# Zhen-Dong/HAWQ

Hardware: AMD Instinct MI355X
Metric: images/sec (higher is better)
Workload: dtype int8

## Files before the change

hawq_amd/csrc/fused_wp.hip:

```cpp
#include <stdio.h>
#include <utility>

#include "common.h"

namespace {

struct WPP {
    const uint8_t *x2, *w3, *w1;
    const int32_t *ctab3, *ctab1;
    const uint16_t *res_in;
    uint16_t *res_out;
    uint8_t *y;
    uint8_t *q_out;
    int q_nib;
    int M, C3;
    int m_id_s, e_id_s, mq, eq, q_hi;
    int y_lo, y_hi, y_planar, y_nib;
    int spb;
    int sub, sW, sHW, dW, dHW;
    int32_t *flags;
    long long *dbgbuf;
};

template <int... Is, class Fn>
__device__ __forceinline__ void sfor_impl(std::integer_sequence<int, Is...>, Fn &&f) {
    (f(std::integral_constant<int, Is>{}), ...);
}
template <int N, class Fn>
__device__ __forceinline__ void sfor(Fn &&f) {
    sfor_impl(std::make_integer_sequence<int, N>{}, f);
}

__device__ __forceinline__ void wp_dma16(const char *src, char *dst) {
    __builtin_amdgcn_global_load_lds((const __attribute__((address_space(1))) void *)src, (__attribute__((address_space(3))) void *)dst, 16, 0, 0);
}
__device__ __forceinline__ void wp_dma4(const char *src, char *dst) {
    __builtin_amdgcn_global_load_lds((const __attribute__((address_space(1))) void *)src, (__attribute__((address_space(3))) void *)dst, 4, 0, 0);
}
template <bool K0>
__device__ __forceinline__ DyNt wp_ctab(const char *ctab, int ch) {
    const v4i t = *reinterpret_cast<const v4i *>(ctab + ch * 16);
    DyNt d;
    d.m = t.x, d.s = K0 ? t.y : (t.y & 31), d.k = K0 ? 0 : (t.y >> 8);
    d.add = (long long)(((unsigned long long)(unsigned)t.w << 32) | (unsigned)t.z);
    return d;
}

template <int C_, int NW_, bool REDUCE_, int MINW_>
struct WPCfg {
    static constexpr int C = C_, NW = NW_, MINW = MINW_;
    static constexpr bool REDUCE = REDUCE_;
    static constexpr int NT = 64 * NW, BM = 32 * NW;
    static constexpr int KC = C / 64;
    static constexpr int CT2 = C / 32;
    static constexpr int RPP = NT / 4;
    static constexpr int W3_BYTES = 64 * C;
    static constexpr int W1_BYTES = REDUCE ? 64 * C : 0;
    static constexpr int STAGE = W3_BYTES + W1_BYTES;
    static constexpr int W3PASS = (64 * KC + RPP - 1) / RPP, W1PASS = REDUCE ? (C + RPP - 1) / RPP : 0;
    static constexpr int CTPASS = NW >= 4 ? 1 : 4 / NW;
    static constexpr int NDMA = W3PASS + W1PASS + CTPASS;
    static constexpr int OFF_CT = 2 * STAGE;
    static constexpr int OFF_STG = OFF_CT + 2 * 1024;
    static constexpr int LDS_BYTES = OFF_STG + NW * 4096;
    static_assert(RPP % 16 == 0 && (NW == 1 || NW == 2 || NW % 4 == 0), "producer passes must cover whole swizzle groups");
};

template <class F, bool TIE, bool CK0, bool QK0 = false>
__global__ __launch_bounds__(F::NT, F::MINW) void expand_wp_kernel(const WPP p) {
    extern __shared__ __attribute__((aligned(16))) char smem[];
    constexpr int MODE_S = TIE ? 2 : 0;
    constexpr int MODE_Q = TIE ? 2 : (QK0 ? 1 : 0);
    constexpr int MODE_C = TIE ? 2 : (CK0 ? 1 : 0);
    constexpr bool K0 = CK0 && !TIE;
    constexpr int C = F::C;
    const int t = threadIdx.x, lane = t & 63, wave = t >> 6, l31 = lane & 31, h = lane >> 5;
    const int pix = blockIdx.x * F::BM + wave * 32 + l31;
    const bool valid = pix < p.M;
    const size_t row = valid ? pix : p.M - 1;
    const int nsl = p.C3 >> 6;
    const int j0 = blockIdx.y * p.spb, j1 = (j0 + p.spb < nsl) ? j0 + p.spb : nsl;
    char *ct = smem + F::OFF_CT;
    const int pix0 = blockIdx.x * F::BM + wave * 32;
    auto srow = [&](int d) -> unsigned {
        d = d < p.M ? d : p.M - 1;
        if constexpr (!F::REDUCE) {
            if (p.sub > 1) {
                const int n = d / p.dHW, r = d - n * p.dHW, y = r / p.dW, x = r - y * p.dW;
                return (unsigned)(n * p.sHW + (y * p.sW + x) * p.sub);
            }
        }
        return (unsigned)d;
    };
    unsigned rsrc[4], xsrc[2];
#pragma unroll
    for (int k = 0; k < 4; ++k) rsrc[k] = srow(pix0 + 8 * k + (lane >> 3));
#pragma unroll
    for (int k = 0; k < 2; ++k) xsrc[k] = srow(pix0 + 16 * k + (lane >> 2));
    asm volatile("" : "+v"(rsrc[0]), "+v"(rsrc[1]), "+v"(rsrc[2]), "+v"(rsrc[3]), "+v"(xsrc[0]), "+v"(xsrc[1]));
    const int prow = t >> 2, pslot = t & 3;
    const int sw = (pslot ^ ((prow >> 2) & 3)) << 4;
    auto issue = [&](int j, int stage) {
        char *dst = smem + stage * F::STAGE;
#pragma unroll
        for (int i = 0; i < F::W3PASS; ++i) {
            const int idx = (i * F::RPP + prow) & (64 * F::KC - 1), first = (i * F::RPP + wave * 16) & (64 * F::KC - 1);
            wp_dma16((const char *)p.w3 + (size_t)(j * 64 + (idx & 63)) * C + (idx >> 6) * 64 + sw, dst + first * 64);
        }
#pragma unroll
        for (int i = 0; i < F::W1PASS; ++i) {
            const int r = (i * F::RPP + prow) & (C - 1), first = (i * F::RPP + wave * 16) & (C - 1);
            wp_dma16((const char *)p.w1 + (size_t)r * p.C3 + j * 64 + sw, dst + F::W3_BYTES + first * 64);
        }
#pragma unroll
        for (int i = 0; i < F::CTPASS; ++i) {
            const int q4 = (wave + i * F::NW) & 3;
            wp_dma4((const char *)p.ctab3 + (size_t)j * 1024 + q4 * 256 + lane * 4, ct + (j & 1) * 1024 + q4 * 256);
        }
    };
    char *stg = smem + F::OFF_STG + wave * 4096;
    const int crow = lane >> 3, cslot = lane & 7;
    unsigned coff[4];
#pragma unroll
    for (int k = 0; k < 4; ++k) {
        const int r = 8 * k + crow;
        coff[k] = rsrc[k] * (unsigned)(p.C3 * 2) + ((cslot ^ (r & 7)) << 4);
    }
    auto dma_res = [&](int j) {
#pragma unroll
        for (int k = 0; k < 4; ++k) wp_dma16((const char *)p.res_in + (coff[k] + (unsigned)(j * 128)), stg + k * 1024);
    };
    const unsigned sl = lds_addr(stg) + l31 * 128;
    const int x7 = l31 & 7;
    v4i xf[F::KC][2];
    {
        const int r2 = lane >> 2, s2 = lane & 3;
#pragma unroll
        for (int kc0 = 0; kc0 < F::KC; kc0 += 2) {
#pragma unroll
            for (int kc = kc0; kc < kc0 + 2 && kc < F::KC; ++kc)
#pragma unroll
                for (int k = 0; k < 2; ++k) {
                    const int r = 16 * k + r2;
                    const size_t gr = xsrc[k];
                    wp_dma16((const char *)p.x2 + gr * C + kc * 64 + ((s2 ^ ((r >> 2) & 3)) << 4), stg + (kc - kc0) * 2048 + k * 1024);
                }
            wait_vmcnt<0>();
#pragma unroll
            for (int kc = kc0; kc < kc0 + 2 && kc < F::KC; ++kc)
#pragma unroll
                for (int ks = 0; ks < 2; ++ks)
                    xf[kc][ks] = *reinterpret_cast<const v4i *>(stg + (kc - kc0) * 2048 + lds_off(l31, 2 * ks + h));
            asm volatile("s_waitcnt lgkmcnt(0)" ::: "memory");
#pragma unroll
            for (int kc = kc0; kc < kc0 + 2 && kc < F::KC; ++kc) pin(xf[kc][0]), pin(xf[kc][1]);
        }
    }
    issue(j0, 0);
    dma_res(j0);
    v16i acc2[F::REDUCE ? F::CT2 : 1];
    if constexpr (F::REDUCE) {
#pragma unroll
        for (int c = 0; c < F::CT2; ++c)
#pragma unroll
            for (int r = 0; r < 16; ++r) acc2[c][r] = 0;
    }
    DyNt dids = dynt_prepare(p.m_id_s, p.e_id_s), dq = dynt_prepare(p.mq, p.eq);
    constexpr bool SC0 = QK0 && !TIE;
    DyS0 dis0 = dys0_prepare(p.m_id_s, p.e_id_s);
    asm volatile("" : "+s"(dids.add), "+s"(dq.add), "+s"(dis0.add));
    const unsigned rowmask = valid ? 0xffffffffu : 0u;
    const int qhi2 = (p.q_hi & 0xffff) | (p.q_hi << 16);
    unsigned oor = 0;
    const int cp = cperm(l31);
    const unsigned a0 = lds_addr(smem) + lds_off(cp, h), a1 = lds_addr(smem) + lds_off(cp, 2 + h);
#ifdef HAWQ_ABLATE
    const bool prof = p.dbgbuf != nullptr;
    long long ph[8] = {0, 0, 0, 0, 0, 0, 0, 0};
    long long tprev = prof ? (long long)__builtin_readcyclecounter() : 0;
#define WP_STAMP(K)                                                    \
    if (prof) {                                                        \
        const long long now = (long long)__builtin_readcyclecounter(); \
        ph[K] += now - tprev;                                          \
        tprev = now;                                                   \
    }
#else
#define WP_STAMP(K)
#endif
    for (int j = j0; j < j1; ++j) {
        const int st = (j - j0) & 1;
        wait_vmcnt<4>();
        __builtin_amdgcn_s_barrier();
        WP_STAMP(0)
        const bool more = j + 1 < j1;
        if (more) issue(j + 1, st ^ 1);
        WP_STAMP(1)
        v16i acc1[2];
#pragma unroll
        for (int r = 0; r < 16; ++r) acc1[0][r] = 0, acc1[1][r] = 0;
        {
            const unsigned b0 = a0 + st * F::STAGE, b1 = a1 + st * F::STAGE;
            v4i wf[2][2];
            wf[0][0] = lds_read16<0>(b0), wf[0][1] = lds_read16<2048>(b0);
            sfor<2 * F::KC>([&](auto SI) {
                constexpr int s = decltype(SI)::value, kc = s >> 1, ks = s & 1, cur = s & 1, nxt = cur ^ 1;
                if constexpr (s + 1 < 2 * F::KC) {
                    constexpr int kn = (s + 1) >> 1;
                    wf[nxt][0] = lds_read16<kn * 4096>(ks ? b0 : b1), wf[nxt][1] = lds_read16<kn * 4096 + 2048>(ks ? b0 : b1);
                    wait_lgkm<2>();
                } else {
                    wait_lgkm<0>();
                }
                pin(wf[cur][0]), pin(wf[cur][1]);
                acc1[0] = __builtin_amdgcn_mfma_i32_32x32x32_i8(wf[cur][0], xf[kc][ks], acc1[0], 0, 0, 0);
                acc1[1] = __builtin_amdgcn_mfma_i32_32x32x32_i8(wf[cur][1], xf[kc][ks], acc1[1], 0, 0, 0);
            });
        }
        WP_STAMP(2)
        if (more) wait_vmcnt<F::NDMA>(); else wait_vmcnt<0>();
        v4i rin[4];
        rin[0] = lds_read16<0>(sl + ((4 * 0 + 2 * h) ^ x7) * 16), rin[1] = lds_read16<0>(sl + ((4 * 0 + 2 * h + 1) ^ x7) * 16);
        rin[2] = lds_read16<0>(sl + ((4 * 1 + 2 * h) ^ x7) * 16), rin[3] = lds_read16<0>(sl + ((4 * 1 + 2 * h + 1) ^ x7) * 16);
        wait_lgkm<0>();
        pin(rin[0]), pin(rin[1]), pin(rin[2]), pin(rin[3]);
        WP_STAMP(3)
        v4i qf[2];
        v4i rout[4];
        {
            const char *ctb = ct + (j & 1) * 1024;
#pragma unroll
            for (int tl = 0; tl < 2; ++tl) {
                int qp[4];
#pragma unroll
                for (int g = 0; g < 4; ++g) {
                    const unsigned w0 = (unsigned)rin[2 * tl + (g >> 1)][(g & 1) * 2], w1 = (unsigned)rin[2 * tl + (g >> 1)][(g & 1) * 2 + 1];
                    const int idin[4] = {(int)(w0 & 0xffffu), (int)(w0 >> 16), (int)(w1 & 0xffffu), (int)(w1 >> 16)};
                    int o[4], qv[4];
#pragma unroll
                    for (int k = 0; k < 4; ++k) {
                        const DyNt dm = wp_ctab<K0>(ctb, 32 * tl + 16 * h + 4 * g + k);
                        const int a = dyadic_mode<MODE_C>(acc1[tl][4 * g + k], dm);
                        const int b = SC0 ? dyadic_s0(idin[k], dis0) : dyadic_mode<MODE_S>(idin[k], dids);
                        o[k] = max(a + b, 0);
                        qv[k] = dyadic_mode<MODE_Q>(o[k], dq);
                    }
                    oor |= ((unsigned)(o[0] | o[1]) | (unsigned)(o[2] | o[3])) & rowmask;
                    rout[2 * tl + (g >> 1)][(g & 1) * 2] = pack2_u16_sat(o[0], o[1]);
                    rout[2 * tl + (g >> 1)][(g & 1) * 2 + 1] = pack2_u16_sat(o[2], o[3]);
                    qp[g] = pack4_min(qv[0], qv[1], qv[2], qv[3], qhi2);
                }
                qf[tl] = v4i{qp[0], qp[1], qp[2], qp[3]};
            }
        }
        WP_STAMP(4)
        if (p.res_out) {
            *reinterpret_cast<v4i *>(stg + l31 * 128 + ((4 * 0 + 2 * h) ^ x7) * 16) = rout[0];
            *reinterpret_cast<v4i *>(stg + l31 * 128 + ((4 * 0 + 2 * h + 1) ^ x7) * 16) = rout[1];
            *reinterpret_cast<v4i *>(stg + l31 * 128 + ((4 * 1 + 2 * h) ^ x7) * 16) = rout[2];
            *reinterpret_cast<v4i *>(stg + l31 * 128 + ((4 * 1 + 2 * h + 1) ^ x7) * 16) = rout[3];
#pragma unroll
            for (int k = 0; k < 4; ++k) {
                const int r = 8 * k + crow;
                const v4i v = *reinterpret_cast<const v4i *>(stg + k * 1024 + lane * 16);
                if (pix0 + r < p.M) *reinterpret_cast<v4i *>((char *)p.res_out + (coff[k] + (unsigned)(j * 128))) = v;
            }
        }
        if constexpr (!F::REDUCE) {
            if (p.q_out && p.q_nib) {
                asm volatile("s_waitcnt lgkmcnt(0)" ::: "memory");
#pragma unroll
                for (int tl = 0; tl < 2; ++tl)
                    *reinterpret_cast<v2i *>(stg + l31 * 32 + 16 * tl + 8 * h) = v2i{qf[tl].x | (qf[tl].y << 4), qf[tl].z | (qf[tl].w << 4)};
                const int r = lane >> 1, s2 = lane & 1;
                const v4i v = *reinterpret_cast<const v4i *>(stg + lane * 16);
                if (pix0 + r < p.M)
                    *reinterpret_cast<v4i *>((char *)p.q_out + (size_t)(pix0 + r) * (p.C3 >> 1) + j * 32 + s2 * 16) = v;
            } else if (p.q_out) {
                asm volatile("s_waitcnt lgkmcnt(0)" ::: "memory");
                *reinterpret_cast<v4i *>(stg + lds_off(l31, h)) = qf[0];
                *reinterpret_cast<v4i *>(stg + lds_off(l31, 2 + h)) = qf[1];
                const int r2 = lane >> 2, s2 = lane & 3;
#pragma unroll
                for (int k = 0; k < 2; ++k) {
                    const int r = 16 * k + r2;
                    const v4i v = *reinterpret_cast<const v4i *>(stg + k * 1024 + lane * 16);
                    if (pix0 + r < p.M)
                        *reinterpret_cast<v4i *>((char *)p.q_out + (size_t)(pix0 + r) * p.C3 + j * 64 + ((s2 ^ ((r >> 2) & 3)) << 4)) = v;
                }
            }
        }
        asm volatile("s_waitcnt lgkmcnt(0)" ::: "memory");
        if (more) dma_res(j + 1);
        WP_STAMP(5)
        if constexpr (F::REDUCE) {
            const unsigned b0 = a0 + st * F::STAGE + F::W3_BYTES, b1 = a1 + st * F::STAGE + F::W3_BYTES;
            v4i wf[2][2];
            wf[0][0] = lds_read16<0>(b0), wf[0][1] = lds_read16<0>(b1);
            sfor<F::CT2>([&](auto CI) {
                constexpr int c = decltype(CI)::value, cur = c & 1, nxt = cur ^ 1;
                if constexpr (c + 1 < F::CT2) {
                    wf[nxt][0] = lds_read16<(c + 1) * 2048>(b0), wf[nxt][1] = lds_read16<(c + 1) * 2048>(b1);
                    wait_lgkm<2>();
                } else {
                    wait_lgkm<0>();
                }
                pin(wf[cur][0]), pin(wf[cur][1]);
                acc2[c] = __builtin_amdgcn_mfma_i32_32x32x32_i8(wf[cur][0], qf[0], acc2[c], 0, 0, 0);
                acc2[c] = __builtin_amdgcn_mfma_i32_32x32x32_i8(wf[cur][1], qf[1], acc2[c], 0, 0, 0);
            });
        }
        WP_STAMP(6)
    }
#ifdef HAWQ_ABLATE
    if (prof && blockIdx.x == 8 && blockIdx.y == 0 && t == 0)
        for (int k = 0; k < 8; ++k) p.dbgbuf[k] = ph[k];
#endif
#undef WP_STAMP
    if ((oor >> 16) != 0) atomicOr(p.flags, 1);
    if constexpr (F::REDUCE) {
        wait_vmcnt<0>();
#pragma unroll
        for (int c = 0; c < F::CT2; ++c) {
            const int ch0 = 32 * c + 16 * h;
            int w[4];
#pragma unroll
            for (int g = 0; g < 4; ++g) {
                int qv[4];
#pragma unroll
                for (int k = 0; k < 4; ++k)
                    qv[k] = med3i(dyadic_mode<MODE_C>(acc2[c][4 * g + k], wp_ctab<K0>((const char *)p.ctab1, ch0 + 4 * g + k)), p.y_lo, p.y_hi);
                w[g] = pack4_fast(qv[0], qv[1], qv[2], qv[3]);
            }
            const v4i ww = {w[0], w[1], w[2], w[3]};
            if (valid && p.y_nib) {
                const v2i nn = {w[0] | (w[1] << 4), w[2] | (w[3] << 4)};
                if (p.y_planar)
                    *reinterpret_cast<v2i *>((char *)p.y + ((size_t)(ch0 >> 5) * p.M + row) * 16 + ((ch0 >> 4) & 1) * 8) = nn;
                else
                    *reinterpret_cast<v2i *>((char *)p.y + row * (C / 2) + (ch0 >> 1)) = nn;
            } else if (valid) {
                if (p.y_planar)
                    *reinterpret_cast<v4i *>((char *)p.y + ((size_t)(ch0 >> 4) * p.M + row) * 16) = ww;
                else
                    *reinterpret_cast<v4i *>((char *)p.y + row * C + ch0) = ww;
            }
        }
    }
}

typedef void (*WPFn)(const WPP);
struct WPInfo { WPFn fn[5]; int c, bm, nt, lds; bool reduce; int ysplit; };
#define WP_ENTRY(F, YS) {{expand_wp_kernel<F, false, false>, expand_wp_kernel<F, false, true>, expand_wp_kernel<F, true, false>, expand_wp_kernel<F, false, true, true>, \
                          expand_wp_kernel<F, false, false, true>}, F::C, F::BM, F::NT, F::LDS_BYTES, F::REDUCE, YS}
using W64 = WPCfg<64, 4, true, 3>;
using W64B = WPCfg<64, 8, true, 3>;
using W128 = WPCfg<128, 4, true, 2>;
using W128B = WPCfg<128, 8, true, 2>;
using W256 = WPCfg<256, 4, true, 1>;
using N64 = WPCfg<64, 4, false, 4>;
using N128 = WPCfg<128, 4, false, 3>;
using N256 = WPCfg<256, 4, false, 3>;
using N512 = WPCfg<512, 4, false, 2>;
const WPInfo kWP[] = {WP_ENTRY(W64, 1), WP_ENTRY(W64B, 1), WP_ENTRY(W128, 1), WP_ENTRY(W128B, 1), WP_ENTRY(W256, 1),
                      WP_ENTRY(N64, 1), WP_ENTRY(N128, 1), WP_ENTRY(N256, 1), WP_ENTRY(N256, 2), WP_ENTRY(N256, 4),
                      WP_ENTRY(N512, 1), WP_ENTRY(N512, 2), WP_ENTRY(N512, 4), WP_ENTRY(N512, 8)};
constexpr int NUM_WP = sizeof(kWP) / sizeof(kWP[0]);

bool wp_expand_ok(const hawq_conv_args &e) {
    return (e.in_pitch == 0 || e.in_pitch == e.Cin) && (e.out_pitch == 0 || e.out_pitch == e.Cout) && e.KH == 1 && e.KW == 1 && e.stride == 1 && e.pad == 0 && e.in_bits == 8 && e.w_bits == 8 && e.fast_tables != 0 && !e.in2 &&
           !e.in_planar && e.epilogue == HAWQ_EPI_RESIDUAL && e.res_in && e.res_in_bits == 16 && (!e.res_out || e.res_out_bits == 16) &&
           e.flags && e.ctab && e.Cout % 64 == 0 && (e.out_bits == 8 || (e.out_bits == 4 && e.q_lo >= 0 && e.q_hi <= 15)) &&
           (e.out_sub < 2 || !e.res_out);
}

int wp_variant(const hawq_expand_reduce_args *a, int nth) {
    const hawq_conv_args &e = a->expand, &r = a->reduce;
    if (!wp_expand_ok(e)) return -1;
    const bool reduce = r.wgt != nullptr;
    if (reduce && e.out_bits != 8) return -1;
    if (reduce && (e.out_sub >= 2 || r.out_sub >= 2)) return -1;
    if (reduce) {
        if (!(r.KH == 1 && r.KW == 1 && r.stride == 1 && r.pad == 0 && r.in_bits == 8 && r.w_bits == 8 && r.fast_tables != 0 && !r.in2)) return -1;
        if (r.epilogue != HAWQ_EPI_REQUANT || !r.ctab || !r.out_q || (r.out_bits != 8 && r.out_bits != 4) || !e.res_out) return -1;
        if (r.out_bits == 4 && (r.q_lo < 0 || r.q_hi > 15)) return -1;
        if (r.Cin != e.Cout || r.Cout != e.Cin || r.N != e.N || r.H != e.H || r.W != e.W) return -1;
    }
    int n = 0;
    for (int i = 0; i < NUM_WP; ++i)
        if (kWP[i].c == e.Cin && kWP[i].reduce == reduce && (e.Cout / 64) % kWP[i].ysplit == 0 && ++n == nth) return i;
    return -1;
}

}

int wp_num_variants(const hawq_expand_reduce_args *a) {
    int n = 0;
    while (wp_variant(a, n + 1) >= 0) ++n;
    return n;
}

int wp_launch(const hawq_expand_reduce_args *a, int nth, void *stream) {
    const int v = wp_variant(a, nth);
    HAWQ_REQUIRE(v >= 0, "hawq_conv_expand_reduce: no wave-private variant %d for this launch", nth);
    const hawq_conv_args &e = a->expand, &r = a->reduce;
    auto e_fast = [](int ek) { return (ek & 0xff) >= 33 && (ek & 0xff) <= 62 && (ek >> 8) >= 0 && (ek >> 8) < 31; };
    HAWQ_REQUIRE(e.mq >= 0 && e_fast(e.eq) && e.m_id_scalar >= 0 && e_fast(e.e_id_scalar), "hawq_conv_expand_reduce: scalar tables outside the fast contract");
    HAWQ_REQUIRE(e.q_lo <= 0, "hawq_conv_expand_reduce: the block-input QuantAct clamp must admit 0");
    const WPInfo &wi = kWP[v];
    WPP p;
    p.x2 = (const uint8_t *)e.in, p.w3 = (const uint8_t *)e.wgt, p.w1 = (const uint8_t *)r.wgt;
    p.ctab3 = e.ctab, p.ctab1 = wi.reduce ? r.ctab : nullptr;
    p.res_in = (const uint16_t *)e.res_in, p.res_out = (uint16_t *)e.res_out;
    p.y = wi.reduce ? (uint8_t *)r.out_q : nullptr;
    p.q_out = wi.reduce ? nullptr : (uint8_t *)e.out_q;
    p.q_nib = !wi.reduce && e.out_bits == 4;
    const int sub = e.out_sub >= 2 ? e.out_sub : 1, hd = (e.H - 1) / sub + 1, wd = (e.W - 1) / sub + 1;
    const long long Msrc = (long long)e.N * e.H * e.W, M = (long long)e.N * hd * wd;
    HAWQ_REQUIRE(M > 0 && Msrc * e.Cout * 2 < (1ll << 32), "hawq_conv_expand_reduce: bad problem size");
    p.M = (int)M, p.C3 = e.Cout;
    p.sub = sub, p.sW = e.W, p.sHW = e.H * e.W, p.dW = wd, p.dHW = hd * wd;
    p.m_id_s = e.m_id_scalar, p.e_id_s = e.e_id_scalar, p.mq = e.mq, p.eq = e.eq, p.q_hi = e.q_hi;
    p.y_lo = wi.reduce ? (r.relu && r.q_lo < 0 ? 0 : r.q_lo) : 0, p.y_hi = wi.reduce ? r.q_hi : 0;
    p.y_planar = wi.reduce ? r.out_planar : 0;
    p.y_nib = wi.reduce && r.out_bits == 4;
    p.spb = (e.Cout / 64) / wi.ysplit;
    p.flags = e.flags;
    p.dbgbuf = nullptr;
#ifdef HAWQ_ABLATE
    static const int dbg_env = HAWQ_DBG_ENV();
    static long long *dbg_dev = nullptr;
    if ((dbg_env & 128) && !dbg_dev) (void)hipMalloc(&dbg_dev, 8 * sizeof(long long));
    if (dbg_env & 128) p.dbgbuf = dbg_dev;
#endif
    static const bool attrs = [] {
        bool good = true;
        for (const WPInfo &k : kWP)
            for (int i = 0; i < 5; ++i)
                good &= hipFuncSetAttribute((const void *)k.fn[i], hipFuncAttributeMaxDynamicSharedMemorySize, k.lds) == hipSuccess;
        return good;
    }();
    HAWQ_REQUIRE(attrs, "hawq_conv_expand_reduce: hipFuncSetAttribute(MaxDynamicSharedMemorySize) failed");
    const int ft = e.fast_tables | (wi.reduce ? r.fast_tables : 0);
    const bool tie = (ft & 4) != 0, ck0 = (e.fast_tables & 8) && (!wi.reduce || (r.fast_tables & 8));
    const bool qk0 = (e.eq >> 8) == 0 && ids0_form(e.e_id_scalar);
    HAWQ_REQUIRE(e.q_hi >= 0 && e.q_hi <= 32767, "hawq_conv_expand_reduce: q_hi outside [0, 32767]");
    hipLaunchKernelGGL(wi.fn[tie ? 2 : (ck0 ? (qk0 ? 3 : 1) : (qk0 ? 4 : 0))], dim3((p.M + wi.bm - 1) / wi.bm, wi.ysplit), dim3(wi.nt), wi.lds, (hipStream_t)stream, p);
    HAWQ_CHECK_HIP(hipGetLastError());
    if (p.dbgbuf) {
        long long hb[8];
        (void)hipStreamSynchronize((hipStream_t)stream);
        (void)hipMemcpy(hb, p.dbgbuf, sizeof(hb), hipMemcpyDeviceToHost);
        fprintf(stderr, "[wave-private C=%d bm=%d reduce=%d ysplit=%d M=%d C3=%d] cycles of wave 0 / workgroup 8 over %d slices: wait+barrier %lld | issue ring DMA %lld | "
                        "GEMM1 %lld | wait + read residual %lld | epilogue %lld | stage + store + residual DMA %lld | GEMM2 %lld\n",
                wi.c, wi.bm, (int)wi.reduce, wi.ysplit, p.M, p.C3, p.spb, hb[0], hb[1], hb[2], hb[3], hb[4], hb[5], hb[6]);
    }
    return 0;
}
```

hawq_amd/engine.py:

```python
from __future__ import annotations

import ctypes as C
import os
import sys
from functools import partial

import numpy as np
import torch

from . import _lib, packing
from . import plan as _plan
from .plan import ChainChoice, StalePlan
from .quant_utils import requant_table, tables_are_fast, tables_fit_fast
from .runner import EventTimer, GraphRunner, _act_range, _i32, two_round_min


RES_VBITS = 20
U16_VBITS = 17


def out_sub_stride(readers) -> int:
    readers = list(readers)
    if not readers:
        return 0
# ... 337 lines not shown
            return True
        if in_bits != c.w_bits or c.band() is None:
            return False
        q.wgt_band, q.in_planar, q.ctab = c.band().data_ptr(), 1, 1
        if is_last:
            q.res_out_bits, q.flags, q.res_out = 16, 1, 1
        return _lib.load().hawq_conv2d_band2_tile(C.byref(q)) != 0

    def _try_fuse(self, a, u, nxt, N, ho, wo, keep):
        if nxt is None or nxt['resize'] or len(nxt['convs']) != 3 or not a.fast_tables:
            return None
        if int(u['name'].split('.')[0][len('stage'):]) not in self.fuse_stages:
            return None
        ent = nxt['convs'][0]
        c = ent['conv']
        if not ent.get('fast', False) or ent['out_bits'] not in (4, 8) or a.in_bits != 8 or a.w_bits != 8:
            return None
        ob = ent['out_bits']
        er = _lib.ExpandReduceArgs()
        C.memmove(C.byref(er.expand), C.byref(a), C.sizeof(a))
        er.expand.out_q, er.expand.out_bits = None, 8
        r = er.reduce
        if c.w_bits != 8 and not hasattr(c, "w8"):
            c.w8 = torch.from_numpy(packing.pack_conv_weight(c.w_host, 8)).to(self.dev)
        r.wgt, r.bias = (c.w if c.w_bits == 8 else c.w8).data_ptr(), c.bias.data_ptr()
        if c.w_bits == 8 and c.k128() is not None:
            r.wgt_k128 = c.k128().data_ptr()
        r.N, r.H, r.W, r.Cin, r.Cout, r.KH, r.KW, r.stride, r.pad = N, ho, wo, c.cin, c.cout, c.kh, c.kw, c.stride, c.pad
        r.in_bits, r.w_bits = 8, 8
        r.m, r.e, r.ctab = ent['m'].data_ptr(), ent['e'].data_ptr(), ent['ctab'].data_ptr()
        r.flags = self.flags.data_ptr()
        r.epilogue, r.relu = _lib.EPI_REQUANT, 1
        r.out_bits, r.q_lo, r.q_hi = ob, ent['rng'][0], ent['rng'][1]
        r.fast_tables = (5 if ent.get('tie', False) else 1) | (8 if ent.get('ck0', False) else 0)
        r.out_q = 1
        if _lib.load().hawq_conv_expand_reduce_variants(C.byref(er)) == 0:
            return None
        out = self._alloc(N * ho * wo * c.cout * ob // 8, torch.uint8)
        r.out_q = out.data_ptr()
        planar = self.planar and self._band_takes(nxt['convs'][1], N, ho, wo, ob, False, nxt)
        r.out_planar = int(planar)
        q = self._alloc(N * ho * wo * c.cin * nxt['a_bits'] // 8, torch.uint8)
        a.out_q = q.data_ptr()
        r1 = _lib.ConvArgs()
        C.memmove(C.byref(r1), C.byref(r), C.sizeof(r1))
        r1.in_, r1.in_bits = q.data_ptr(), nxt['a_bits']
        r1.wgt, r1.w_bits = c.w.data_ptr(), c.w_bits
        r1.wgt_k128 = c.k128().data_ptr() if (c.k128() is not None and c.w_bits == nxt['a_bits']) else None
        pair = _FusedPair(er, a, r1, self.stream.cuda_stream, self._ws)
        keep += [out, er, q, r1, pair]
        return pair, out, ob, planar

    def _try_solo(self, a, u, keep):
        if not a.fast_tables or a.in2 or os.environ.get("HAWQ_NO_SOLO"):
            return None
        er = _lib.ExpandReduceArgs()
        C.memmove(C.byref(er.expand), C.byref(a), C.sizeof(a))
        if _lib.load().hawq_conv_expand_reduce_variants(C.byref(er)) == 0:
            return None
        pair = _FusedPair(er, a, None, self.stream.cuda_stream, self._ws)
        keep += [er, pair]
        return pair

    def _alloc(self, n, dtype):
        return torch.empty(n, dtype=dtype, device=self.dev)

    def _build(self, N, H, W):
        self._build_plan(N, H, W)
        if not os.environ.get("HAWQ_KEEP_PACKED"):
            self._release_unused_weights()

    def _release_unused_weights(self):
        lib = _lib.load()
        n, nb2, ng2 = lib.hawq_conv2d_num_tiles(), lib.hawq_conv2d_num_band2_tiles(), lib.hawq_conv2d_num_gemm2_tiles()
        band_ids, gemm_ids = range(n - ng2 - nb2 + 1, n - ng2 + 1), range(n - ng2 + 1, n + 1)
        args = []
        for e in (self.subs or [self]):
            args += list(e._conv_args)
            for pr in e._er_args:
                if not pr.fused:
                    args += [pr.expand] + ([pr.reduce] if pr.reduce is not None else [])
        live_band = {a.wgt_band for a in args if a.wgt_band and (a.tile in band_ids or a.tile == 0)}
        live_k128 = {ptr for a in args if (a.tile in gemm_ids or a.tile == 0) for ptr in (a.wgt_k128, a.wgt2_k128) if ptr}
        every = []
        for e in (self.subs or [self]):
            every += list(e._conv_args)
            for pr in e._er_args:
                every += [pr.expand, pr.er.expand, pr.er.reduce] + ([pr.reduce] if pr.reduce is not None else [])
        for a in every:
            if a.wgt_band and a.wgt_band not in live_band:
                a.wgt_band = None
            if a.wgt_k128 and a.wgt_k128 not in live_k128:
                a.wgt_k128 = None
            if a.wgt2_k128 and a.wgt2_k128 not in live_k128:
                a.wgt2_k128 = None
        convs = [c for u in self.P['units'] for c in [ent['conv'] for ent in u['convs']] + ([u['ident']] if u['resize'] else [])]
        self.packed_weight_bytes = 0
        for c in convs:
            wb, wk = c._w_band, c._w_k128
            c.release(wb is not None and wb.data_ptr() not in live_band, wk is not None and wk.data_ptr() not in live_k128)
            self.packed_weight_bytes += sum(t.numel() for t in (c._w_band, c._w_k128) if t is not None)

    def _build_plan(self, N, H, W):
        self._plan_on = bool(self.plan) and int(self.plan.get("batch", -1)) == N and not self.keep_acc
        self.chains = max(1, self.chains_req)
        if self._plan_on:
            try:
# ... 258 lines not shown
                    planar_next = bool(a.fast_tables) and self.planar and self._band_takes(u['convs'][ci + 1], N, ho, wo, xb_next,
                                                                                            ci + 1 == len(u['convs']) - 1, u)
                    a.out_planar = int(planar_next)
                else:
                    a.epilogue = _lib.EPI_RESIDUAL
                    if u['resize']:
                        ic = u['ident']
                        a.in2, a.wgt2, a.bias2 = qa.data_ptr(), ic.w.data_ptr(), ic.bias.data_ptr()
                        if u['a_bits'] == ic.w_bits and ic.k128() is not None:
                            a.wgt2_k128 = ic.k128().data_ptr()
                        a.H2, a.W2, a.Cin2, a.stride2 = h, w, ic.cin, (1 if sub_in else ic.stride)
                        a.in2_bits, a.w2_bits = u['a_bits'], ic.w_bits
                        a.m_id, a.e_id = u['m_id'].data_ptr(), u['e_id'].data_ptr()
                    else:
                        a.res_in, a.res_in_bits = res.data_ptr(), res_bits_in
                        a.m_id_scalar, a.e_id_scalar = u['m_id_s'], u['e_id_s']
                    need_res = (nxt is None) or (not nxt['resize'])
                    new_res = self._alloc(N * ho * wo * c.cout, rdt) if need_res else None
                    if sub_out:
                        a.out_sub = sub_out
                        qh, qw = out_sub_extent(ho, sub_out), out_sub_extent(wo, sub_out)
                    else:
                        qh, qw = ho, wo
                    if new_res is not None:
                        a.res_out, a.res_out_bits = new_res.data_ptr(), self.res_bits
                        self.res_taps[u['name']] = (new_res, (N, ho, wo, c.cout))
                    new_qa = None
                    if nxt is not None:
                        a.out_bits = nxt['a_bits']
                        a.q_lo, a.q_hi, a.mq, a.eq = nxt['a_rng'][0], nxt['a_rng'][1], nxt['mq'], nxt['eq']
                    keep.append(new_res)
                if self.keep_acc:
                    self._add_acc_tap(ops, keep, a, tap_name, N, ho, wo, c.cout)
                    if ci == len(u['convs']) - 1 and u['resize']:
                        self._add_ident_tap(ops, keep, u, qa, N, h, w, ho, wo)
                keep.append(a)
                fz = self._try_fuse(a, u, nxt, N, ho, wo, keep) if (ci == len(u['convs']) - 1 and not self.keep_acc) else None
                if fz is None and ci == len(u['convs']) - 1 and nxt is not None:
                    new_qa = self._alloc(N * qh * qw * c.cout * nxt['a_bits'] // 8, torch.uint8)
                    a.out_q = new_qa.data_ptr()
                    keep.append(new_qa)
                if fz is not None:
                    pair, fout, fbits, fplanar = fz
                    fused_in = (fout, fbits, fplanar)
                    self._er_args.append(pair)
                    self._er_names.append(tap_name)
                    ops.next_name = tap_name + "+" + nxt['name'] + ".quant_convbn1"
                    ops.append(pair)
                    continue
                solo = self._try_solo(a, u, keep) if (ci == len(u['convs']) - 1 and not self.keep_acc) else None
                if solo is not None:
                    self._er_args.append(solo)
                    self._er_names.append(tap_name + "@solo")
                    ops.next_name = tap_name
                    ops.append(solo)
                    continue
                self._conv_args.append(a)
                self._conv_names.append(tap_name)
                self._conv_ops.append(_ConvLaunch(a, self._ws, sp))
                ops.next_name = tap_name + ("+identity" if (a.in2 is not None) else "")
                ops.append(self._conv_ops[-1])
                if ci < len(u['convs']) - 1:
                    x_in, x_bits, hin, win, x_planar = x_next, xb_next, ho, wo, planar_next
            res, qa, h, w = new_res, new_qa, qh, qw
            res_bits_in = self.res_bits
        cl = units[-1]['convs'][-1]['conv'].cout
        qf = self._alloc(N * cl, torch.int8)
        pooled = self._alloc(N * cl, torch.int32) if self.keep_acc else None
        if pooled is not None:
            self.acc_taps['final_pool'] = (pooled, (N, cl))
        o = P['out']
        ops.append(partial(_lib.call, "hawq_avgpool_requant", res.data_ptr(), self.res_bits, N, h * w, cl, qf.data_ptr(),
                           ptr(pooled), o['mq'], o['eq'], o['rng'][0], o['rng'][1], sp))
        fc = P['fc']
        if fc['k'] != cl:
            raise RuntimeError("FC input width does not match the last stage")
        self.logits = logits_view if logits_view is not None else torch.empty(N, fc['nout'], dtype=torch.float32, device=dev)
        a = _lib.ConvArgs()
        a.in_, a.wgt, a.bias = qf.data_ptr(), fc['w'].data_ptr(), fc['bias'].data_ptr()
        a.N, a.H, a.W, a.Cin, a.Cout, a.KH, a.KW, a.stride, a.pad = N, 1, 1, fc['k'], fc['nout_p'], 1, 1, 1, 0
        a.in_bits, a.w_bits = 8, 8
        a.epilogue = _lib.EPI_DEQUANT
        a.out_f32, a.fscale, a.ldo, a.n_valid = self.logits.data_ptr(), fc['fscale'].data_ptr(), fc['nout'], fc['nout']
        if self.keep_acc:
            self._add_acc_tap(ops, keep, a, 'quant_output', N, 1, 1, fc['nout_p'])
        ops.next_name = "quant_output"
        if _lib.load().hawq_fc_dequant_ok(N, fc['k'], fc['nout_p']) and not os.environ.get("HAWQ_NO_FC2"):
            ops.append(partial(_lib.call, "hawq_fc_dequant", qf.data_ptr(), fc['w'].data_ptr(), fc['bias'].data_ptr(), fc['fscale'].data_ptr(),
                               self.logits.data_ptr(), N, fc['k'], fc['nout_p'], fc['nout'], fc['nout'], sp))
        else:
            self._conv_ops.append(_ConvLaunch(a, self._ws, sp))
            ops.append(self._conv_ops[-1])
            self._conv_args.append(a)
            self._conv_names.append("quant_output")
        keep += [qf, pooled, a]
        self._ops, self._keep, self._batch = ops, keep, (N, H, W)
        self._graph = None
        if self.autotune and not self.keep_acc:
            ch = _plan.decode(fixed, chain, self._conv_names, len(self._er_args), int(_lib.load().hawq_conv2d_num_tiles()), self._variant_counts())
            self._apply_choice(self._time_choice(ch) if ch.tiles is None else ch)

    def _add_acc_tap(self, ops, keep, a, name, N, ho, wo, cout):
        acc = self._alloc(N * ho * wo * cout, torch.int32)
        r = _lib.ConvArgs()
        C.memmove(C.byref(r), C.byref(a), C.sizeof(r))
        r.in2 = None
        r.epilogue, r.out_acc = _lib.EPI_RAW, acc.data_ptr()
# ... 246 lines not shown
```

Measured before the change: 104,200.

## Fuse downsample identity conv into wave-private expand kernel via dual GEMM

Adds a DUAL variant of the wave-private expand kernel that computes the downsample/identity 1x1 conv (second input and weights, optionally strided) alongside the main expand GEMM. The two MFMA streams are interleaved in one loop, and each has its own requant table. This lets blocks whose last conv carries an identity branch (in2) take the solo fused path instead of the generic conv kernel. It also switches output stores to nontemporal in that variant, at the cost of more LDS, more registers and a full vmcnt wait per slice.

```diff
diff --git a/hawq_amd/csrc/fused_wp.hip b/hawq_amd/csrc/fused_wp.hip
--- a/hawq_amd/csrc/fused_wp.hip
+++ b/hawq_amd/csrc/fused_wp.hip
@@ -1,4 +1,5 @@
 #include <stdio.h>
+#include <stdlib.h>
 #include <utility>
 
 #include "common.h"
@@ -7,7 +8,8 @@
 
 struct WPP {
     const uint8_t *x2, *w3, *w1;
-    const int32_t *ctab3, *ctab1;
+    const uint8_t *xid, *wid;
+    const int32_t *ctab3, *ctab1, *ctab_id;
     const uint16_t *res_in;
     uint16_t *res_out;
     uint8_t *y;
@@ -18,6 +20,7 @@
     int y_lo, y_hi, y_planar, y_nib;
     int spb;
     int sub, sW, sHW, dW, dHW;
+    int s2, sW2, sHW2;
     int32_t *flags;
     long long *dbgbuf;
 };
@@ -36,6 +39,10 @@
 }
 __device__ __forceinline__ void wp_dma4(const char *src, char *dst) {
     __builtin_amdgcn_global_load_lds((const __attribute__((address_space(1))) void *)src, (__attribute__((address_space(3))) void *)dst, 4, 0, 0);
+}
+template <bool NT>
+__device__ __forceinline__ void wp_store(v4i *dst, const v4i &v) {
+    if constexpr (NT) __builtin_nontemporal_store(v, dst); else *dst = v;
 }
 template <bool K0>
 __device__ __forceinline__ DyNt wp_ctab(const char *ctab, int ch) {
@@ -46,25 +53,38 @@
     return d;
 }
 
-template <int C_, int NW_, bool REDUCE_, int MINW_>
+template <int C_, int NW_, bool REDUCE_, int MINW_, int K2_ = 0>
 struct WPCfg {
-    static constexpr int C = C_, NW = NW_, MINW = MINW_;
-    static constexpr bool REDUCE = REDUCE_;
+    static constexpr int C = C_, NW = NW_, MINW = MINW_, K2 = K2_;
+    static constexpr bool REDUCE = REDUCE_, DUAL = K2_ > 0;
     static constexpr int NT = 64 * NW, BM = 32 * NW;
     static constexpr int KC = C / 64;
     static constexpr int CT2 = C / 32;
     static constexpr int RPP = NT / 4;
     static constexpr int W3_BYTES = 64 * C;
     static constexpr int W1_BYTES = REDUCE ? 64 * C : 0;
-    static constexpr int STAGE = W3_BYTES + W1_BYTES;
+    static constexpr int KC2 = K2 / 64;
+    static constexpr int WID_BYTES = 64 * K2;
+    static constexpr int OFF_WID = W3_BYTES + W1_BYTES;
+    static constexpr int STAGE = W3_BYTES + W1_BYTES + WID_BYTES;
     static constexpr int W3PASS = (64 * KC + RPP - 1) / RPP, W1PASS = REDUCE ? (C + RPP - 1) / RPP : 0;
+    static constexpr int WIDPASS = (64 * KC2 + RPP - 1) / RPP;
     static constexpr int CTPASS = NW >= 4 ? 1 : 4 / NW;
-    static constexpr int NDMA = W3PASS + W1PASS + CTPASS;
+    static constexpr int NDMA = W3PASS + W1PASS + WIDPASS + (DUAL ? 2 : 1) * CTPASS;
     static constexpr int OFF_CT = 2 * STAGE;
-    static constexpr int OFF_STG = OFF_CT + 2 * 1024;
+    static constexpr int OFF_STG = OFF_CT + (DUAL ? 4 : 2) * 1024;
     static constexpr int LDS_BYTES = OFF_STG + NW * 4096;
     static_assert(RPP % 16 == 0 && (NW == 1 || NW == 2 || NW % 4 == 0), "producer passes must cover whole swizzle groups");
+    static_assert(K2 % 64 == 0 && (!DUAL || 64 * KC2 >= RPP), "an identity pass may not be wider than the identity slice");
 };
+
+constexpr int wp_merge(int i, int S1, int S2) {
+    int a = 0, b = 0;
+    for (int n = 0; n < i; ++n) {
+        if (b >= S2 || (a < S1 && a * S2 <= b * S1)) ++a; else ++b;
+    }
+    return (b >= S2 || (a < S1 && a * S2 <= b * S1)) ? a : 256 + b;
+}
 
 template <class F, bool TIE, bool CK0, bool QK0 = false>
 __global__ __launch_bounds__(F::NT, F::MINW) void expand_wp_kernel(const WPP p) {
@@ -117,6 +137,18 @@
             const int q4 = (wave + i * F::NW) & 3;
             wp_dma4((const char *)p.ctab3 + (size_t)j * 1024 + q4 * 256 + lane * 4, ct + (j & 1) * 1024 + q4 * 256);
         }
+        if constexpr (F::DUAL) {
+#pragma unroll
+            for (int i = 0; i < F::WIDPASS; ++i) {
+                const int idx = (i * F::RPP + prow) & (64 * F::KC2 - 1), first = (i * F::RPP + wave * 16) & (64 * F::KC2 - 1);
+                wp_dma16((const char *)p.wid + (size_t)(j * 64 + (idx & 63)) * F::K2 + (idx >> 6) * 64 + sw, dst + F::OFF_WID + first * 64);
+            }
+#pragma unroll
+            for (int i = 0; i < F::CTPASS; ++i) {
+                const int q4 = (wave + i * F::NW) & 3;
+                wp_dma4((const char *)p.ctab_id + (size_t)j * 1024 + q4 * 256 + lane * 4, ct + 2048 + (j & 1) * 1024 + q4 * 256);
+            }
+        }
     };
     char *stg = smem + F::OFF_STG + wave * 4096;
     const int crow = lane >> 3, cslot = lane & 7;
@@ -156,8 +188,43 @@
             for (int kc = kc0; kc < kc0 + 2 && kc < F::KC; ++kc) pin(xf[kc][0]), pin(xf[kc][1]);
         }
     }
+    v4i xid[F::DUAL ? F::KC2 : 1][2];
+    if constexpr (F::DUAL) {
+        const int r2 = lane >> 2, s2 = lane & 3;
+        unsigned xsrc2[2];
+#pragma unroll
+        for (int k = 0; k < 2; ++k) {
+            int d = pix0 + 16 * k + r2;
+            d = d < p.M ? d : p.M - 1;
+            if (p.s2 > 1) {
+                const int n = d / p.dHW, r = d - n * p.dHW, y = r / p.dW, x = r - y * p.dW;
+                d = n * p.sHW2 + (y * p.sW2 + x) * p.s2;
+            }
+            xsrc2[k] = (unsigned)d;
+        }
+#pragma unroll
+        for (int kc0 = 0; kc0 < F::KC2; kc0 += 2) {
+#pragma unroll
+            for (int kc = kc0; kc < kc0 + 2 && kc < F::KC2; ++kc)
+#pragma unroll
+                for (int k = 0; k < 2; ++k) {
+                    const int r = 16 * k + r2;
+                    const size_t gr = xsrc2[k];
+                    wp_dma16((const char *)p.xid + gr * F::K2 + kc * 64 + ((s2 ^ ((r >> 2) & 3)) << 4), stg + (kc - kc0) * 2048 + k * 1024);
+                }
+            wait_vmcnt<0>();
+#pragma unroll
+            for (int kc = kc0; kc < kc0 + 2 && kc < F::KC2; ++kc)
+#pragma unroll
+                for (int ks = 0; ks < 2; ++ks)
+                    xid[kc][ks] = *reinterpret_cast<const v4i *>(stg + (kc - kc0) * 2048 + lds_off(l31, 2 * ks + h));
+            asm volatile("s_waitcnt lgkmcnt(0)" ::: "memory");
+#pragma unroll
+            for (int kc = kc0; kc < kc0 + 2 && kc < F::KC2; ++kc) pin(xid[kc][0]), pin(xid[kc][1]);
+        }
+    }
     issue(j0, 0);
-    dma_res(j0);
+    if constexpr (!F::DUAL) dma_res(j0);
     v16i acc2[F::REDUCE ? F::CT2 : 1];
     if constexpr (F::REDUCE) {
 #pragma unroll
@@ -165,10 +232,15 @@
 #pragma unroll
             for (int r = 0; r < 16; ++r) acc2[c][r] = 0;
     }
-    DyNt dids = dynt_prepare(p.m_id_s, p.e_id_s), dq = dynt_prepare(p.mq, p.eq);
+    DyNt dids{}, dq = dynt_prepare(p.mq, p.eq);
     constexpr bool SC0 = QK0 && !TIE;
-    DyS0 dis0 = dys0_prepare(p.m_id_s, p.e_id_s);
-    asm volatile("" : "+s"(dids.add), "+s"(dq.add), "+s"(dis0.add));
+    DyS0 dis0{};
+    if constexpr (!F::DUAL) {
+        dids = dynt_prepare(p.m_id_s, p.e_id_s), dis0 = dys0_prepare(p.m_id_s, p.e_id_s);
+        asm volatile("" : "+s"(dids.add), "+s"(dq.add), "+s"(dis0.add));
+    } else {
+        asm volatile("" : "+s"(dq.add));
+    }
     const unsigned rowmask = valid ? 0xffffffffu : 0u;
     const int qhi2 = (p.q_hi & 0xffff) | (p.q_hi << 16);
     unsigned oor = 0;
@@ -189,16 +261,44 @@
 #endif
     for (int j = j0; j < j1; ++j) {
         const int st = (j - j0) & 1;
-        wait_vmcnt<4>();
+        if constexpr (F::DUAL) wait_vmcnt<0>(); else wait_vmcnt<4>();
         __builtin_amdgcn_s_barrier();
         WP_STAMP(0)
         const bool more = j + 1 < j1;
         if (more) issue(j + 1, st ^ 1);
         WP_STAMP(1)
-        v16i acc1[2];
+        v16i acc1[2], accid[F::DUAL ? 2 : 1];
 #pragma unroll
         for (int r = 0; r < 16; ++r) acc1[0][r] = 0, acc1[1][r] = 0;
-        {
+        if constexpr (F::DUAL) {
+#pragma unroll
+            for (int r = 0; r < 16; ++r) accid[0][r] = 0, accid[1][r] = 0;
+            const unsigned b0 = a0 + st * F::STAGE, b1 = a1 + st * F::STAGE;
+            constexpr int S1 = 2 * F::KC, S2 = 2 * F::KC2;
+            auto frag = [&](auto EI, v4i &f0, v4i &f1) {
+                constexpr int e = decltype(EI)::value, g = e >> 8, s = e & 255, off = (g ? F::OFF_WID : 0) + (s >> 1) * 4096;
+                f0 = lds_read16<off>((s & 1) ? b1 : b0), f1 = lds_read16<off + 2048>((s & 1) ? b1 : b0);
+            };
+            v4i wf[2][2];
+            frag(std::integral_constant<int, wp_merge(0, S1, S2)>{}, wf[0][0], wf[0][1]);
+            sfor<S1 + S2>([&](auto SI) {
+                constexpr int i = decltype(SI)::value, e = wp_merge(i, S1, S2), g = e >> 8, s = e & 255, cur = i & 1, nxt = cur ^ 1;
+                if constexpr (i + 1 < S1 + S2) {
+                    frag(std::integral_constant<int, wp_merge(i + 1, S1, S2)>{}, wf[nxt][0], wf[nxt][1]);
+                    wait_lgkm<2>();
+                } else {
+                    wait_lgkm<0>();
+                }
+                pin(wf[cur][0]), pin(wf[cur][1]);
+                if constexpr (g == 0) {
+                    acc1[0] = __builtin_amdgcn_mfma_i32_32x32x32_i8(wf[cur][0], xf[s >> 1][s & 1], acc1[0], 0, 0, 0);
+                    acc1[1] = __builtin_amdgcn_mfma_i32_32x32x32_i8(wf[cur][1], xf[s >> 1][s & 1], acc1[1], 0, 0, 0);
+                } else {
+                    accid[0] = __builtin_amdgcn_mfma_i32_32x32x32_i8(wf[cur][0], xid[s >> 1][s & 1], accid[0], 0, 0, 0);
+                    accid[1] = __builtin_amdgcn_mfma_i32_32x32x32_i8(wf[cur][1], xid[s >> 1][s & 1], accid[1], 0, 0, 0);
+                }
+            });
+        } else {
             const unsigned b0 = a0 + st * F::STAGE, b1 = a1 + st * F::STAGE;
             v4i wf[2][2];
             wf[0][0] = lds_read16<0>(b0), wf[0][1] = lds_read16<2048>(b0);
@@ -217,12 +317,14 @@
             });
         }
         WP_STAMP(2)
-        if (more) wait_vmcnt<F::NDMA>(); else wait_vmcnt<0>();
-        v4i rin[4];
-        rin[0] = lds_read16<0>(sl + ((4 * 0 + 2 * h) ^ x7) * 16), rin[1] = lds_read16<0>(sl + ((4 * 0 + 2 * h + 1) ^ x7) * 16);
-        rin[2] = lds_read16<0>(sl + ((4 * 1 + 2 * h) ^ x7) * 16), rin[3] = lds_read16<0>(sl + ((4 * 1 + 2 * h + 1) ^ x7) * 16);
-        wait_lgkm<0>();
-        pin(rin[0]), pin(rin[1]), pin(rin[2]), pin(rin[3]);
+        v4i rin[F::DUAL ? 1 : 4];
+        if constexpr (!F::DUAL) {
+            if (more) wait_vmcnt<F::NDMA>(); else wait_vmcnt<0>();
+            rin[0] = lds_read16<0>(sl + ((4 * 0 + 2 * h) ^ x7) * 16), rin[1] = lds_read16<0>(sl + ((4 * 0 + 2 * h + 1) ^ x7) * 16);
+            rin[2] = lds_read16<0>(sl + ((4 * 1 + 2 * h) ^ x7) * 16), rin[3] = lds_read16<0>(sl + ((4 * 1 + 2 * h + 1) ^ x7) * 16);
+            wait_lgkm<0>();
+            pin(rin[0]), pin(rin[1]), pin(rin[2]), pin(rin[3]);
+        }
         WP_STAMP(3)
         v4i qf[2];
         v4i rout[4];
@@ -233,14 +335,22 @@
                 int qp[4];
 #pragma unroll
                 for (int g = 0; g < 4; ++g) {
-                    const unsigned w0 = (unsigned)rin[2 * tl + (g >> 1)][(g & 1) * 2], w1 = (unsigned)rin[2 * tl + (g >> 1)][(g & 1) * 2 + 1];
-                    const int idin[4] = {(int)(w0 & 0xffffu), (int)(w0 >> 16), (int)(w1 & 0xffffu), (int)(w1 >> 16)};
+                    int idin[4];
+                    if constexpr (!F::DUAL) {
+                        const unsigned w0 = (unsigned)rin[2 * tl + (g >> 1)][(g & 1) * 2], w1 = (unsigned)rin[2 * tl + (g >> 1)][(g & 1) * 2 + 1];
+                        idin[0] = (int)(w0 & 0xffffu), idin[1] = (int)(w0 >> 16), idin[2] = (int)(w1 & 0xffffu), idin[3] = (int)(w1 >> 16);
+                    }
                     int o[4], qv[4];
+                    if constexpr (F::DUAL) __builtin_amdgcn_sched_barrier(0);
 #pragma unroll
                     for (int k = 0; k < 4; ++k) {
                         const DyNt dm = wp_ctab<K0>(ctb, 32 * tl + 16 * h + 4 * g + k);
                         const int a = dyadic_mode<MODE_C>(acc1[tl][4 * g + k], dm);
-                        const int b = SC0 ? dyadic_s0(idin[k], dis0) : dyadic_mode<MODE_S>(idin[k], dids);
+                        int b;
+                        if constexpr (F::DUAL)
+                            b = dyadic_mode<MODE_C>(accid[tl][4 * g + k], wp_ctab<K0>(ctb + 2048, 32 * tl + 16 * h + 4 * g + k));
+                        else
+                            b = SC0 ? dyadic_s0(idin[k], dis0) : dyadic_mode<MODE_S>(idin[k], dids);
                         o[k] = max(a + b, 0);
                         qv[k] = dyadic_mode<MODE_Q>(o[k], dq);
                     }
@@ -262,7 +372,7 @@
             for (int k = 0; k < 4; ++k) {
                 const int r = 8 * k + crow;
                 const v4i v = *reinterpret_cast<const v4i *>(stg + k * 1024 + lane * 16);
-                if (pix0 + r < p.M) *reinterpret_cast<v4i *>((char *)p.res_out + (coff[k] + (unsigned)(j * 128))) = v;
+                if (pix0 + r < p.M) wp_store<F::DUAL>(reinterpret_cast<v4i *>((char *)p.res_out + (coff[k] + (unsigned)(j * 128))), v);
             }
         }
         if constexpr (!F::REDUCE) {
@@ -285,12 +395,14 @@
                     const int r = 16 * k + r2;
                     const v4i v = *reinterpret_cast<const v4i *>(stg + k * 1024 + lane * 16);
                     if (pix0 + r < p.M)
-                        *reinterpret_cast<v4i *>((char *)p.q_out + (size_t)(pix0 + r) * p.C3 + j * 64 + ((s2 ^ ((r >> 2) & 3)) << 4)) = v;
+                        wp_store<F::DUAL>(reinterpret_cast<v4i *>((char *)p.q_out + (size_t)(pix0 + r) * p.C3 + j * 64 + ((s2 ^ ((r >> 2) & 3)) << 4)), v);
                 }
             }
         }
         asm volatile("s_waitcnt lgkmcnt(0)" ::: "memory");
-        if (more) dma_res(j + 1);
+        if constexpr (!F::DUAL) {
+            if (more) dma_res(j + 1);
+        }
         WP_STAMP(5)
         if constexpr (F::REDUCE) {
             const unsigned b0 = a0 + st * F::STAGE + F::W3_BYTES, b1 = a1 + st * F::STAGE + F::W3_BYTES;
@@ -349,9 +461,11 @@
 }
 
 typedef void (*WPFn)(const WPP);
-struct WPInfo { WPFn fn[5]; int c, bm, nt, lds; bool reduce; int ysplit; };
+struct WPInfo { WPFn fn[5]; int c, k2, bm, nt, lds; bool reduce; int ysplit; };
 #define WP_ENTRY(F, YS) {{expand_wp_kernel<F, false, false>, expand_wp_kernel<F, false, true>, expand_wp_kernel<F, true, false>, expand_wp_kernel<F, false, true, true>, \
-                          expand_wp_kernel<F, false, false, true>}, F::C, F::BM, F::NT, F::LDS_BYTES, F::REDUCE, YS}
+                          expand_wp_kernel<F, false, false, true>}, F::C, 0, F::BM, F::NT, F::LDS_BYTES, F::REDUCE, YS}
+#define WP_DUAL_ENTRY(F, YS) {{expand_wp_kernel<F, false, false>, expand_wp_kernel<F, false, true>, expand_wp_kernel<F, true, false>, nullptr, nullptr}, \
+                              F::C, F::K2, F::BM, F::NT, F::LDS_BYTES, F::REDUCE, YS}
 using W64 = WPCfg<64, 4, true, 3>;
 using W64B = WPCfg<64, 8, true, 3>;
 using W128 = WPCfg<128, 4, true, 2>;
@@ -361,14 +475,23 @@
 using N128 = WPCfg<128, 4, false, 3>;
 using N256 = WPCfg<256, 4, false, 3>;
 using N512 = WPCfg<512, 4, false, 2>;
+using D128 = WPCfg<128, 4, false, 2, 256>;
 const WPInfo kWP[] = {WP_ENTRY(W64, 1), WP_ENTRY(W64B, 1), WP_ENTRY(W128, 1), WP_ENTRY(W128B, 1), WP_ENTRY(W256, 1),
                       WP_ENTRY(N64, 1), WP_ENTRY(N128, 1), WP_ENTRY(N256, 1), WP_ENTRY(N256, 2), WP_ENTRY(N256, 4),
-                      WP_ENTRY(N512, 1), WP_ENTRY(N512, 2), WP_ENTRY(N512, 4), WP_ENTRY(N512, 8)};
+                      WP_ENTRY(N512, 1), WP_ENTRY(N512, 2), WP_ENTRY(N512, 4), WP_ENTRY(N512, 8),
+                      WP_DUAL_ENTRY(D128, 1), WP_DUAL_ENTRY(D128, 2)};
 constexpr int NUM_WP = sizeof(kWP) / sizeof(kWP[0]);
 
+bool wp_dual_ok(const hawq_conv_args &e) {
+    const char *off = getenv("HAWQ_NO_WP_DUAL");
+    return !(off && *off) && e.wgt2 && e.ctab_id && e.in2_bits == 8 && e.w2_bits == 8 && e.stride2 >= 1 && e.H2 >= 1 && e.W2 >= 1 &&
+           (e.H2 - 1) / e.stride2 + 1 == e.H && (e.W2 - 1) / e.stride2 + 1 == e.W &&
+           !e.res_in && e.out_sub < 2 && e.out_bits == 8;
+}
+
 bool wp_expand_ok(const hawq_conv_args &e) {
-    return (e.in_pitch == 0 || e.in_pitch == e.Cin) && (e.out_pitch == 0 || e.out_pitch == e.Cout) && e.KH == 1 && e.KW == 1 && e.stride == 1 && e.pad == 0 && e.in_bits == 8 && e.w_bits == 8 && e.fast_tables != 0 && !e.in2 &&
-           !e.in_planar && e.epilogue == HAWQ_EPI_RESIDUAL && e.res_in && e.res_in_bits == 16 && (!e.res_out || e.res_out_bits == 16) &&
+    return (e.in_pitch == 0 || e.in_pitch == e.Cin) && (e.out_pitch == 0 || e.out_pitch == e.Cout) && e.KH == 1 && e.KW == 1 && e.stride == 1 && e.pad == 0 && e.in_bits == 8 && e.w_bits == 8 && e.fast_tables != 0 &&
+           !e.in_planar && e.epilogue == HAWQ_EPI_RESIDUAL && (e.in2 ? wp_dual_ok(e) : (e.res_in && e.res_in_bits == 16)) && (!e.res_out || e.res_out_bits == 16) &&
            e.flags && e.ctab && e.Cout % 64 == 0 && (e.out_bits == 8 || (e.out_bits == 4 && e.q_lo >= 0 && e.q_hi <= 15)) &&
            (e.out_sub < 2 || !e.res_out);
 }
@@ -385,9 +508,11 @@
         if (r.out_bits == 4 && (r.q_lo < 0 || r.q_hi > 15)) return -1;
         if (r.Cin != e.Cout || r.Cout != e.Cin || r.N != e.N || r.H != e.H || r.W != e.W) return -1;
     }
+    const int k2 = e.in2 ? e.Cin2 : 0;
+    if (e.in2 && k2 <= 0) return -1;
     int n = 0;
     for (int i = 0; i < NUM_WP; ++i)
-        if (kWP[i].c == e.Cin && kWP[i].reduce == reduce && (e.Cout / 64) % kWP[i].ysplit == 0 && ++n == nth) return i;
+        if (kWP[i].c == e.Cin && kWP[i].k2 == k2 && kWP[i].reduce == reduce && (e.Cout / 64) % kWP[i].ysplit == 0 && ++n == nth) return i;
     return -1;
 }
 
@@ -404,11 +529,13 @@
     HAWQ_REQUIRE(v >= 0, "hawq_conv_expand_reduce: no wave-private variant %d for this launch", nth);
     const hawq_conv_args &e = a->expand, &r = a->reduce;
     auto e_fast = [](int ek) { return (ek & 0xff) >= 33 && (ek & 0xff) <= 62 && (ek >> 8) >= 0 && (ek >> 8) < 31; };
-    HAWQ_REQUIRE(e.mq >= 0 && e_fast(e.eq) && e.m_id_scalar >= 0 && e_fast(e.e_id_scalar), "hawq_conv_expand_reduce: scalar tables outside the fast contract");
+    const bool dual = e.in2 != nullptr;
+    HAWQ_REQUIRE(e.mq >= 0 && e_fast(e.eq) && (dual || (e.m_id_scalar >= 0 && e_fast(e.e_id_scalar))), "hawq_conv_expand_reduce: scalar tables outside the fast contract");
     HAWQ_REQUIRE(e.q_lo <= 0, "hawq_conv_expand_reduce: the block-input QuantAct clamp must admit 0");
     const WPInfo &wi = kWP[v];
     WPP p;
     p.x2 = (const uint8_t *)e.in, p.w3 = (const uint8_t *)e.wgt, p.w1 = (const uint8_t *)r.wgt;
+    p.xid = (const uint8_t *)e.in2, p.wid = (const uint8_t *)e.wgt2, p.ctab_id = dual ? e.ctab_id : nullptr;
     p.ctab3 = e.ctab, p.ctab1 = wi.reduce ? r.ctab : nullptr;
     p.res_in = (const uint16_t *)e.res_in, p.res_out = (uint16_t *)e.res_out;
     p.y = wi.reduce ? (uint8_t *)r.out_q : nullptr;
@@ -419,6 +546,8 @@
     HAWQ_REQUIRE(M > 0 && Msrc * e.Cout * 2 < (1ll << 32), "hawq_conv_expand_reduce: bad problem size");
     p.M = (int)M, p.C3 = e.Cout;
     p.sub = sub, p.sW = e.W, p.sHW = e.H * e.W, p.dW = wd, p.dHW = hd * wd;
+    p.s2 = dual ? e.stride2 : 1, p.sW2 = e.W2, p.sHW2 = e.H2 * e.W2;
+    HAWQ_REQUIRE(!dual || (long long)e.N * e.H2 * e.W2 * e.Cin2 < (1ll << 32), "hawq_conv_expand_reduce: bad problem size");
     p.m_id_s = e.m_id_scalar, p.e_id_s = e.e_id_scalar, p.mq = e.mq, p.eq = e.eq, p.q_hi = e.q_hi;
     p.y_lo = wi.reduce ? (r.relu && r.q_lo < 0 ? 0 : r.q_lo) : 0, p.y_hi = wi.reduce ? r.q_hi : 0;
     p.y_planar = wi.reduce ? r.out_planar : 0;
@@ -436,13 +565,13 @@
         bool good = true;
         for (const WPInfo &k : kWP)
             for (int i = 0; i < 5; ++i)
-                good &= hipFuncSetAttribute((const void *)k.fn[i], hipFuncAttributeMaxDynamicSharedMemorySize, k.lds) == hipSuccess;
+                good &= !k.fn[i] || hipFuncSetAttribute((const void *)k.fn[i], hipFuncAttributeMaxDynamicSharedMemorySize, k.lds) == hipSuccess;
         return good;
     }();
     HAWQ_REQUIRE(attrs, "hawq_conv_expand_reduce: hipFuncSetAttribute(MaxDynamicSharedMemorySize) failed");
     const int ft = e.fast_tables | (wi.reduce ? r.fast_tables : 0);
     const bool tie = (ft & 4) != 0, ck0 = (e.fast_tables & 8) && (!wi.reduce || (r.fast_tables & 8));
-    const bool qk0 = (e.eq >> 8) == 0 && ids0_form(e.e_id_scalar);
+    const bool qk0 = !dual && (e.eq >> 8) == 0 && ids0_form(e.e_id_scalar);
     HAWQ_REQUIRE(e.q_hi >= 0 && e.q_hi <= 32767, "hawq_conv_expand_reduce: q_hi outside [0, 32767]");
     hipLaunchKernelGGL(wi.fn[tie ? 2 : (ck0 ? (qk0 ? 3 : 1) : (qk0 ? 4 : 0))], dim3((p.M + wi.bm - 1) / wi.bm, wi.ysplit), dim3(wi.nt), wi.lds, (hipStream_t)stream, p);
     HAWQ_CHECK_HIP(hipGetLastError());
diff --git a/hawq_amd/engine.py b/hawq_amd/engine.py
--- a/hawq_amd/engine.py
+++ b/hawq_amd/engine.py
@@ -413,7 +413,7 @@
         return pair, out, ob, planar
 
     def _try_solo(self, a, u, keep):
-        if not a.fast_tables or a.in2 or os.environ.get("HAWQ_NO_SOLO"):
+        if not a.fast_tables or os.environ.get("HAWQ_NO_SOLO"):
             return None
         er = _lib.ExpandReduceArgs()
         C.memmove(C.byref(er.expand), C.byref(a), C.sizeof(a))
@@ -778,7 +778,7 @@
                 if solo is not None:
                     self._er_args.append(solo)
                     self._er_names.append(tap_name + "@solo")
-                    ops.next_name = tap_name
+                    ops.next_name = tap_name + ("+identity" if (a.in2 is not None) else "")
                     ops.append(solo)
                     continue
                 self._conv_args.append(a)
```

Measured after the change: 102,600. -1.5%, worse.
